# vghuy17ck1/svt-av1-psyex

Measured on AMD Instinct MI355X. Metric: ME+RD-cost Mpixels/s (2160p10 preset-6), higher is better.
Workload: dtype u8 SAD / i32 transforms; 1 GPU; 3840x2160 10-bit synthetic pan sequence, preset 6 (M6) search controls at qp 35; step = 16 pictures (4 current pictures x ref distance 1,2,4,8; R=2): open-loop ME of all 2040 b64 + full-pel pred + RD chain (64x64,32x32,16x16 DCT_DCT, 10-bit, b quantizer; qcoeff + recon + scalars written); 3 picture sets alternate from step to step

## Files before the change

svt-av1-psyex_amd/csrc/me_kernel.hip:

```cpp
#include <hip/hip_runtime.h>
#include <stdint.h>
#include <string.h>
#include "me_kernel.h"
#include "wave_ops.h"

#ifdef SVT_HIP_ME_PROFILE
struct Prof { uint32_t *acc; unsigned long long last; int step; };
#define SVT_HIP_ME_PROFILE_LDS (48 * 4)
#define PROF_DECL Prof prof_; prof_.acc = reinterpret_cast<uint32_t *>(g_lds + lay.total); if (threadIdx.x < 48) prof_.acc[threadIdx.x] = 0; prof_.last = __builtin_readcyclecounter(); prof_.step = 0; Prof *prof = &prof_
#define PROF_STEP(s) (prof->step = (s))
#define PROFS(i) PROF((i) + prof->step)
#define PROF(i) do { const unsigned long long t_ = __builtin_readcyclecounter(); if (threadIdx.x == 0) atomicAdd(&prof->acc[i], (uint32_t)(t_ - prof->last)); prof->last = t_; } while (0)
#define PROF_FLUSH(ptr) do { __builtin_amdgcn_fence(__ATOMIC_RELEASE, "wavefront"); if (threadIdx.x < 48) atomicAdd((unsigned long long *)(ptr) + threadIdx.x, (unsigned long long)prof->acc[threadIdx.x]); } while (0)
#define PROF_PARAM , Prof *prof
#define PROF_ARG , prof
#else
#define PROF_DECL do { } while (0)
#define PROF(i) do { } while (0)
#define PROFS(i) do { } while (0)
#define PROF_STEP(s) do { } while (0)
#define PROF_FLUSH(ptr) do { } while (0)
#define SVT_HIP_ME_PROFILE_LDS 0
#define PROF_PARAM
#define PROF_ARG
// ... 757 lines not shown
    best        = k < best ? k : best;
}

__device__ __attribute__((noinline)) void stage_clamped(uint8_t *win, const uint8_t *pix0, uint32_t stride, int min_x, int max_x, int min_y, int max_y, int wx0, int wy0,
                                                        int pitch, int rows) {
    for (int i = threadIdx.x; i < pitch * rows; i += kThreads) {
        const int row = i / pitch, cb = i - row * pitch;
        const int x = imin(imax(wx0 + cb, min_x), max_x), y = imin(imax(wy0 + row, min_y), max_y);
        win[row * pitch + cb] = pix0[x + (long long)y * stride];
    }
}

constexpr int kMeInFlight = 4;
constexpr int kMeOrdBits = 12;
__device__ __forceinline__ void run_me_searches(Shared &sh, CParams &p, const MeReq *list, int count, uint32_t *bsad, uint32_t *bmv, int r0n PROF_PARAM) {
    const int lane = threadIdx.x;
    const int sub  = (p.cfg.me_search_method == 0);
    const int nrow = sub ? 4 : 8, rstep = sub ? 2 : 1;
    const int g = lane >> 4, pu = lane & 15;
    const int bx = (pu & 1) | ((pu >> 1) & 2), by = ((pu >> 1) & 1) | ((pu >> 2) & 2);
    const uint8_t *srow = &LDS(sh.src64)[bx * 16];
    for (int mi = 0; mi < count; mi++) {
        MeReq m;
        {
            const MeReq &mm = list[mi];
            m.pix0 = uni_ptr(mm.pix0); m.stride = uni(mm.stride);
            m.ox = (int16_t)uni((uint32_t)mm.ox); m.oy = (int16_t)uni((uint32_t)mm.oy); m.sa_w = (int16_t)uni((uint32_t)mm.sa_w); m.sa_h = (int16_t)uni((uint32_t)mm.sa_h);
            m.li = (uint8_t)uni(mm.li); m.ri = (uint8_t)uni(mm.ri); m.probe = 0; m.pad = 0;
            m.min_x = (int16_t)uni((uint32_t)mm.min_x); m.max_x = (int16_t)uni((uint32_t)mm.max_x); m.min_y = (int16_t)uni((uint32_t)mm.min_y); m.max_y = (int16_t)uni((uint32_t)mm.max_y);
        }
        u64 b8[4] = {~0ull, ~0ull, ~0ull, ~0ull}, b16 = ~0ull, b32 = ~0ull, b64 = ~0ull;
        const int W = m.sa_w, H = m.sa_h;
        int       tw = W, th = H;
        auto me_pitch = [](int shift, int ww) { return ((shift + ww - 1 + 64 + 15) & ~15) + 16; };
        auto wbytes = [&](int ww, int hh) { return (uint32_t)me_pitch(0, ww) * (uint32_t)(hh - 1 + 64); };
        while (th > 1 && (wbytes(tw, th) > (uint32_t)kWinBytes || tw * th > (1 << kMeOrdBits))) th = (th + 1) >> 1;
        while (tw > 8 && (wbytes(tw, th) > (uint32_t)kWinBytes || tw * th > (1 << kMeOrdBits))) tw = ((tw >> 1) + 7) & ~7;
        for (int y0 = 0; y0 < H; y0 += th)
            for (int x0 = 0; x0 < W; x0 += tw) {
                const int w = imin(tw, W - x0), h = imin(th, H - y0);
                const uint8_t *gwin  = m.pix0 + (m.ox + x0) + (long long)(m.oy + y0) * m.stride;
                const int pitch = me_pitch(0, w);
                const int rows        = h - 1 + 64;
                const int vec_per_row = pitch >> 4;
                const float vpr_rcp   = rcp_of((uint32_t)vec_per_row);
                wave_sync();
                const int wx0 = m.ox + x0, wy0 = m.oy + y0;
                if (m.ox + x0 >= m.min_x && m.ox + x0 + w - 1 + 63 <= m.max_x && wy0 >= m.min_y && wy0 + rows - 1 <= m.max_y) {
                    const int nvec = vec_per_row * rows;
                    for (int b0 = 0; b0 < nvec; b0 += kMeInFlight * kThreads) {
                        const int base = b0 + lane;
                        int  k[kMeInFlight];
                        V4   v[kMeInFlight];
#pragma unroll
                        for (int j = 0; j < kMeInFlight; j++) {
                            if (b0 + j * kThreads < nvec) {
                                k[j] = imin(base + j * kThreads, nvec - 1);
                                const int row = (int)div_by_rcp((uint32_t)k[j], vpr_rcp), c = k[j] - row * vec_per_row;
                                const V4U q4 = *reinterpret_cast<GV4U *>(reinterpret_cast<uintptr_t>(gwin + (long long)row * m.stride + c * 16));
                                v[j] = V4{q4.x, q4.y, q4.z, q4.w};
                            }
                        }
#pragma unroll
                        for (int j = 0; j < kMeInFlight; j++)
                            if (b0 + j * kThreads < nvec) *reinterpret_cast<V4 *>(&LDS(sh.win)[k[j] * 16]) = v[j];
                    }
                } else {
                    stage_clamped(LDS(sh.win), m.pix0, m.stride, m.min_x, m.max_x, m.min_y, m.max_y, wx0, wy0, pitch, rows);
                }
                wave_sync();
                PROF(46);
                const int ng = (w + 3) >> 2;
                uint32_t k8[4] = {~0u, ~0u, ~0u, ~0u}, k16 = ~0u, k32 = ~0u, k64 = ~0u;
                const int kshift = kMeOrdBits + sub;
                for (int y = 0; y < h; y += 4) {
                    const bool live = y + g < h;
                    const int  yy   = live ? y + g : h - 1;
                    const uint8_t *wrow = &LDS(sh.win)[(yy + by * 16) * pitch + bx * 16];
                    const uint32_t ord0 = (uint32_t)(yy * w);
                    for (int gq = 0; gq < ng; gq++) {
                        const uint8_t *wp = wrow + 4 * gq;
                        u64 acc[4] = {0, 0, 0, 0};
#pragma unroll
                        for (int half = 0; half < 2; half++)
#pragma unroll
                            for (int k = 0; k < 8; k++) {
                                if (k < nrow) {
                                    const int r = 8 * half + k * rstep;
                                    const uint32_t *wr = reinterpret_cast<const uint32_t *>(wp + r * pitch);
                                    const uint32_t d0 = wr[0], d1 = wr[1], d2 = wr[2], d3 = wr[3], d4 = wr[4];
                                    const uint4 sv = *reinterpret_cast<const uint4 *>(srow + ((by * 16 + r) >> sh.cshift) * kSrc64Pitch);
                                    acc[2 * half] = __builtin_amdgcn_qsad_pk_u16_u8(((u64)d1 << 32) | d0, sv.x, acc[2 * half]);
                                    acc[2 * half] = __builtin_amdgcn_qsad_pk_u16_u8(((u64)d2 << 32) | d1, sv.y, acc[2 * half]);
                                    acc[2 * half + 1] = __builtin_amdgcn_qsad_pk_u16_u8(((u64)d3 << 32) | d2, sv.z, acc[2 * half + 1]);
                                    acc[2 * half + 1] = __builtin_amdgcn_qsad_pk_u16_u8(((u64)d4 << 32) | d3, sv.w, acc[2 * half + 1]);
                                }
                            }
#pragma unroll
                        for (int i = 0; i < 4; i++) {
                            const int x = 4 * gq + i;
                            uint32_t v8[4];
#pragma unroll
                            for (int j = 0; j < 4; j++) v8[j] = (uint32_t)((acc[j] >> (16 * i)) & 0xFFFF);
                            const uint32_t v16 = (v8[0] + v8[1]) + (v8[2] + v8[3]);
                            const uint32_t v32 = quad_sum(v16);
                            const uint32_t v64 = row16_sum_of_quads(v32);
                            if (x < w && live) {
                                const uint32_t ord = ord0 + (uint32_t)x;
#pragma unroll
                                for (int j = 0; j < 4; j++) k8[j] = umin32(k8[j], (v8[j] << kshift) | ord);
                                k16 = umin32(k16, (v16 << kshift) | ord);
                                k32 = umin32(k32, (v32 << kshift) | ord);
                                k64 = umin32(k64, (v64 << kshift) | ord);
                            }
                        }
                    }
                }
                PROF(47);
                const float w_rcp = rcp_of((uint32_t)w);
                auto fold = [&](u64 &best, uint32_t k) {
                    k = umin32(k, (uint32_t)__shfl_xor((int)k, 16, 64));
                    k = umin32(k, (uint32_t)__shfl_xor((int)k, 32, 64));
                    if (k != ~0u) {
                        const uint32_t ordl = k & ((1u << kMeOrdBits) - 1u), ty = div_by_rcp(ordl, w_rcp), tx = ordl - ty * (uint32_t)w;
                        upd(best, k >> kMeOrdBits, (uint32_t)((y0 + (int)ty) * W + (x0 + (int)tx)));
                    }
                };
#pragma unroll
                for (int j = 0; j < 4; j++) fold(b8[j], k8[j]);
                fold(b16, k16); fold(b32, k32); fold(b64, k64);
            }
        uint32_t *rs_ = bsad + ((m.li ? r0n : 0) + m.ri) * 85, *rm_ = bmv + ((m.li ? r0n : 0) + m.ri) * 85;
        auto merge = [&](int n, u64 k) {
            const uint32_t sad = (uint32_t)(k >> 32);
            if (k != ~0ull && sad < rs_[n]) {
                const uint32_t ord = (uint32_t)k;
                const int      yy = (int)(ord / (uint32_t)W), xx = (int)(ord - (uint32_t)yy * (uint32_t)W);
                rs_[n] = sad;
                rm_[n] = ((uint32_t)(m.oy + yy) << 16) | (uint16_t)(m.ox + xx);
            }
        };
        if (g == 0) {
#pragma unroll
            for (int j = 0; j < 4; j++) merge(21 + 4 * pu + j, b8[j]);
            merge(5 + pu, b16);
            if ((pu & 3) == 0) merge(1 + (pu >> 2), b32);
            if (pu == 0) merge(0, b64);
        }
        wave_sync();
    }
}


__device__ __forceinline__ bool searched(CParams &p, int li) { return p.desc.temporal_layer_index > 0 || li == 0; }

__device__ void set_hme_all(St &st, CParams &p, int lvl, int li, int ri, int x, int y, uint32_t sad) {
    for (int h = 0; h < p.cfg.num_hme_sa_h; h++)
        for (int w = 0; w < p.cfg.num_hme_sa_w; w++) {
            st.hx[lvl][li][ri][w][h] = (int16_t)x;
            st.hy[lvl][li][ri][w][h] = (int16_t)y;
            st.hs[lvl][li][ri][w][h] = sad;
        }
}

template <class P> __host__ __device__ __forceinline__ void hme_l0_area(P &p, int li, int ri, uint32_t dist, int mvx, int mvy, int &sa_w, int &sa_h) {
    auto &c = p.cfg;
    struct { SvtHipSearchAreaMinMax hme_l0_sa; } st;
    st.hme_l0_sa.sa_min.width = (uint16_t)c.hme_l0_sa.sa_min.width; st.hme_l0_sa.sa_min.height = (uint16_t)c.hme_l0_sa.sa_min.height;
    st.hme_l0_sa.sa_max.width = (uint16_t)c.hme_l0_sa.sa_max.width; st.hme_l0_sa.sa_max.height = (uint16_t)c.hme_l0_sa.sa_max.height;
    if (c.enable_me_sr_adjustment && c.distance_based_hme_resizing) {
        int is_hor = 1, is_ver = 1, is_still = 0;
        if (c.reduce_hme_l0_sr_th_min && c.reduce_hme_l0_sr_th_max && (li || ri)) {
            is_ver   = iabs(mvx) < c.reduce_hme_l0_sr_th_min && iabs(mvy) > c.reduce_hme_l0_sr_th_max;
            is_hor   = iabs(mvx) > c.reduce_hme_l0_sr_th_max && iabs(mvy) < c.reduce_hme_l0_sr_th_min;
            is_still = iabs(mvx) < c.reduce_hme_l0_sr_th_min * 3 && iabs(mvy) < c.reduce_hme_l0_sr_th_min * 3;
        }
        int xo = is_hor ? 1 : 2, yo = is_ver ? 1 : 2;
        if (c.enable_me_sr_adjustment == 2 && is_still) xo = yo = 4;
        st.hme_l0_sa.sa_min.width  = (uint16_t)(st.hme_l0_sa.sa_min.width / (xo + ri));
        st.hme_l0_sa.sa_min.height = (uint16_t)(st.hme_l0_sa.sa_min.height / (yo + ri));
        st.hme_l0_sa.sa_max.width  = (uint16_t)(st.hme_l0_sa.sa_max.width / (xo + ri));
        st.hme_l0_sa.sa_max.height = (uint16_t)(st.hme_l0_sa.sa_max.height / (yo + ri));
    }
    const int f = (int)scaled_distance(dist);
    int       w = (int16_t)(st.hme_l0_sa.sa_min.width / c.num_hme_sa_w);
    w           = (int16_t)imin(((w * f) + 15) & ~15, ((st.hme_l0_sa.sa_max.width / c.num_hme_sa_w) + 15) & ~15);
    int h       = (int16_t)(st.hme_l0_sa.sa_min.height / c.num_hme_sa_h);
    h           = (int16_t)imin(h * f, st.hme_l0_sa.sa_max.height / c.num_hme_sa_h);
    sa_w        = w;
    sa_h        = h;
}
__device__ void hme_l0_search_area(const St &cst, CParams &p, int li, int ri, uint32_t dist, int &sa_w, int &sa_h) {
    hme_l0_area(p, li, ri, dist, cst.hx[0][0][0][0][0], cst.hy[0][0][0][0][0], sa_w, sa_h);
}

template <class P> __host__ __device__ __forceinline__ void prehme_size(P &p, int li, int ri, int sri, int &sa_w, int &sa_h) {
    auto &c = p.cfg;
    const uint32_t f = scaled_distance(ref_distance(p, li, ri));
    sa_w = (int16_t)(uint16_t)imin((int)(c.prehme_sa_cfg[sri].sa_min.width * f), c.prehme_sa_cfg[sri].sa_max.width);
    sa_h = (int16_t)(uint16_t)imin((int)(c.prehme_sa_cfg[sri].sa_min.height * f), c.prehme_sa_cfg[sri].sa_max.height);
}
__device__ __forceinline__ SearchGeo prehme_geometry(CParams &p, int li, int ri, int sri, uint32_t org_x, uint32_t org_y) {
    int sa_w, sa_h;
    prehme_size(p, li, ri, sri, sa_w, sa_h);
    CPlane &rp = p.ref[li][ri].lvl[0];
    const int ox16 = (int16_t)org_x >> 2, oy16 = (int16_t)org_y >> 2;
    int ox = -(int16_t)(sa_w >> 1), oy = -(int16_t)(sa_h >> 1);
    clip_axis(ox16, ox, sa_w, rp.org_x - 1, rp.width);
    clip_axis(oy16, oy, sa_h, rp.org_y - 1, rp.height);
    SearchGeo g = {ox, oy, sa_w, sa_h};
    return g;
}

__device__ __forceinline__ SearchGeo hme_level_geometry(CParams &p, int level, CPlane &rp, int org_x, int org_y, int sa_w, int sa_h, int cx, int cy, int sr_w, int sr_h) {
    sa_w = (int16_t)((sa_w + 7) & ~7);
    int pad_w, pad_h, ox, oy;
    if (level == 2) { pad_w = pad_h = 63; } else { pad_w = rp.org_x - 1; pad_h = rp.org_y - 1; }
    if (level == 0) {
        ox = -(int16_t)((sa_w * p.cfg.num_hme_sa_w) >> 1) + (int16_t)(sa_w * sr_w);
        oy = -(int16_t)((sa_h * p.cfg.num_hme_sa_h) >> 1) + (int16_t)(sa_h * sr_h);
    } else {
        ox = -(sa_w >> 1) + cx;
        oy = -(sa_h >> 1) + cy;
    }
    clip_axis(org_x, ox, sa_w, pad_w, rp.width);
    sa_w = (sa_w < 8) ? sa_w : (sa_w & ~7);
    clip_axis(org_y, oy, sa_h, pad_h, rp.height);
    SearchGeo g = {ox, oy, sa_w, sa_h};
    return g;
}

struct HmeGeom { int16_t ox, oy; };

__device__ HmeGeom push_hme_level(St &st, CParams &p, int level, CPlane &rp, int org_x, int org_y, int bw, int bh,
                                  int sa_w, int sa_h, int cx, int cy, int sr_w, int sr_h, int slot = -1) {
    const SearchGeo sg = hme_level_geometry(p, level, rp, org_x, org_y, sa_w, sa_h, cx, cy, sr_w, sr_h);
    push_hme_req(st, p, level, rp, org_x, org_y, bw, bh, sg.ox, sg.oy, sg.sa_w, sg.sa_h, 0, slot);
    HmeGeom g = {(int16_t)sg.ox, (int16_t)sg.oy};
    return g;
}

__device__ __forceinline__ void key_to_result(u64 key, int full, uint32_t &sad, int &x, int &y) {
    sad = (uint32_t)(key >> 32);
    if ((uint32_t)key == 0xffffffffu) { x = 0; y = 0; }
    else { y = (int)((key >> 16) & 0xFFFF); x = (int)(key & 0xFFFF); }
    if (!full) sad *= 2;
}

__device__ __forceinline__ void push_zz_req(St &st, CPlane &rp, int dx, int dy, int slot = -1) {
    push_req(st, plane_at(rp, (int)st.org_x + dx, (int)st.org_y + dy), rp.stride, 1, 1, (int)st.b64_w, (int)st.b64_h >> 1, 2, 2, 0, slot);
}

}


#ifndef SVT_ME_CTRL_PRIO
#define SVT_ME_CTRL_PRIO 2
#endif
#define CTRL_PRIO(x) __builtin_amdgcn_s_setprio(x)

constexpr size_t kPersistBytes = (offsetof(St, req) + 15) & ~(size_t)15;
template <int MODE>
__device__ __forceinline__ void me_b64_body(const MeBatchHeader *__restrict__ ghdr, const MeKernelParams *__restrict__ gparams, const uint32_t launch_flags) {
    St     &st = *reinterpret_cast<St *>(g_lds);
    typedef const SVT_CONST_AS MeBatchHeader CHeader;
    CHeader  &hdr = *(CHeader *)ghdr;
    const int tid = threadIdx.x;
    const int       cshift = (int)hdr.cshift;
    const bool      has_dense = hdr.dense != nullptr;
    const LdsLayout lay    = lds_layout((int)hdr.n_slot, cshift, has_dense ? 1 : 0, MODE);
    uint32_t *const bsad = reinterpret_cast<uint32_t *>(g_lds + lay.bsad);
    uint32_t *const bmv  = reinterpret_cast<uint32_t *>(g_lds + lay.bmv);
    const MeDenseSlot *const dense_lds = has_dense ? reinterpret_cast<const MeDenseSlot *>(g_lds + lay.dense) : nullptr;
    uint32_t n_hit = 0, n_miss = 0;
    Shared sh = {st, lay.src64, lay.src32, lay.src16, lay.win, cshift};

    uint32_t xcc = 0;
    asm volatile("s_getreg_b32 %0, hwreg(HW_REG_XCC_ID)" : "=s"(xcc));
    xcc &= 7;
    int queue_probe = 0;
    constexpr int kList = 0;
    const bool list_mode = (launch_flags & 1u) != 0;
    const uint32_t n_total = hdr.job_base[hdr.n_pictures];
    uint32_t share_next = 0, share_end = 0, share_step = 1;
    if (MODE != kMeFull && !list_mode) {
        if (gridDim.x >= SVT_HIP_ME_QUEUES) {
            const uint32_t q = blockIdx.x % SVT_HIP_ME_QUEUES;
            share_step = (gridDim.x - q + SVT_HIP_ME_QUEUES - 1) / SVT_HIP_ME_QUEUES;
            share_next = hdr.queue_begin[q] + blockIdx.x / SVT_HIP_ME_QUEUES;
            share_end  = hdr.queue_begin[q + 1];
        } else {
            share_step = gridDim.x; share_next = blockIdx.x; share_end = n_total;
        }
    }
    auto fetch_job = [&]() {
        int job = -1;
        if (list_mode) {
            const uint32_t n = __hip_atomic_load(&hdr.queue_head[SVT_HIP_ME_LIST_COUNT(kList)], __ATOMIC_RELAXED, __HIP_MEMORY_SCOPE_AGENT);
            if (__hip_atomic_load(&hdr.queue_head[SVT_HIP_ME_LIST_CURSOR(kList)], __ATOMIC_RELAXED, __HIP_MEMORY_SCOPE_AGENT) >= n) return job;
            const uint32_t k = atomicAdd(&hdr.queue_head[SVT_HIP_ME_LIST_CURSOR(kList)], 1u);
            if (k < n) job = (int)hdr.lists[kList][k];
            return job;
        }
        if (MODE != kMeFull) {
            if (share_next < share_end) { job = (int)share_next; share_next += share_step; }
            return job;
// ... 478 lines not shown
            const bool mine = tid < 8 && li < nl && ri < d.num_of_ref_pic_to_search[li] && !(dep && ((li == 0 && ri == 0) != (gi == 0))) && st.do_ref[li][ri];
            MeReq m = {};
            if (mine) {
                CPlane &rp = p.ref[li][ri].lvl[2];
                int16_t  cx = st.me_cx[li][ri], cy = st.me_cy[li][ri];
                const uint32_t dist = mctf ? (uint16_t)ref_distance(p, li, ri) : (uint16_t)scaled_distance(ref_distance(p, li, ri));
                int16_t sa_w = (int16_t)imin((int)(c.me_sa.sa_min.width * dist), c.me_sa.sa_max.width);
                int16_t sa_h = (int16_t)imin((int)(c.me_sa.sa_min.height * dist), c.me_sa.sa_max.height);
                if (c.mv_sa_adj_enabled && (!c.mv_sa_adj_nearest_ref_only || ri == 0)) {
                    if (iabs(st.hme_sc_x[li][ri]) > c.mv_sa_adj_mv_size_th) sa_w = (int16_t)(sa_w * c.mv_sa_adj_sa_multiplier);
                    if (iabs(st.hme_sc_y[li][ri]) > c.mv_sa_adj_mv_size_th) sa_h = (int16_t)(sa_h * c.mv_sa_adj_sa_multiplier);
                }
                { const uint32_t q = (uint32_t)(int)sa_w / st.sr_divisor[li][ri]; sa_w = (int16_t)(((q > 1u ? q : 1u) + 7) & ~7u); }
                { const uint32_t q = (uint32_t)(int)sa_h / st.sr_divisor[li][ri]; sa_h = (int16_t)(q > 3u ? q : 3u); }
                const int16_t h0 = sa_h, w0 = sa_w;
                u64 best_hme_sad = ~0ull;
                if (c.me_early_exit_th) {
                    if (st.zz_sad[li][ri] < c.me_early_exit_th / 6) sa_w = sa_h = 1;
                } else {
                    int accurate = 1;
                    const int k2 = st.c00_req[li][ri];
                    if (k2) {
                        const uint32_t zero = (uint32_t)(st.req_key[k2 - 2] >> 32) << 1;
                        const uint32_t hme  = (uint32_t)(st.req_key[k2 - 1] >> 32) << 1;
                        if (zero <= hme) cx = cy = 0;
                        best_hme_sad = hme;
                        if (cx == 0 && cy == 0) accurate = 0;
                    }
                    if (c.enable_me_sr_adjustment == 2) {
                        if ((accurate && best_hme_sad < 24 * 24) || (d.is_ref && st.hme_sad64[li][ri] < 24 * 24)) sa_h = (int16_t)(sa_h / 2);
                        if ((li || ri) && BEST_SAD(0, 0)[0] < 5000 && sa_h == h0 && sa_w == w0) { sa_h = (int16_t)(sa_h >> 1); sa_w = (int16_t)(sa_w >> 1); }
                    }
                }
                m.pix0 = plane_at(rp, (int)st.org_x, (int)st.org_y); m.stride = rp.stride;
                m.min_x = (int16_t)(-rp.org_x - (int)st.org_x); m.max_x = (int16_t)(rp.width + rp.org_x - 1 - (int)st.org_x);
                m.min_y = (int16_t)(-rp.org_y - (int)st.org_y); m.max_y = (int16_t)(rp.height + rp.org_y - 1 - (int)st.org_y);
                m.li = (uint8_t)li; m.ri = (uint8_t)ri; m.pad = 0;
                m.sa_w = sa_w; m.sa_h = sa_h;
                m.ox = cx; m.oy = cy;
                m.probe = (c.me_8x8_var_enabled && sa_w * sa_h > 24) ? 1 : 0;
            }
            const bool probe = mine && m.probe;
            const u64  mask = __ballot(mine), pmask = __ballot(probe), below = (1ull << tid) - 1ull;
            if (mine) st.me[__popcll(mask & below)] = m;
            if (probe) { MeReq pr = m; pr.sa_w = pr.sa_h = 1; st.me_probe[__popcll(pmask & below)] = pr; }
            if (tid == 0) { st.nme = __popcll(mask); st.nprobe = __popcll(pmask); }
        };
        auto main_pre = [&]() {
            if (tid < 64) {
                const int pic_w = (int16_t)d.aligned_width, pic_h = (int16_t)d.aligned_height;
                for (int i = 0; i < st.nme; i++) {
                    const MeReq m = st.me[i];
                    int16_t sa_w = m.sa_w, sa_h = m.sa_h;
                    const int cx = m.ox, cy = m.oy;
                    if (m.probe) {
                        const uint32_t mean = BEST_SAD(m.li, m.ri)[0] / 64;
                        const int32_t  dd   = (int32_t)BEST_SAD(m.li, m.ri)[21 + tid] - (int32_t)mean;
                        const uint32_t var  = wave_sum((uint32_t)(dd * dd)) / 64;
                        if (var > c.me_sr_mult2_th) { sa_w = (int16_t)((imax(1, sa_w * 3 / 2) + 7) & ~7); sa_h = (int16_t)imax(1, sa_h * 3 / 2); }
                        if (var < c.me_sr_div4_th) { sa_w = (int16_t)((imax(1, sa_w >> 2) + 7) & ~7); sa_h = (int16_t)imax(3, imax(1, sa_h >> 2)); }
                        else if (var < c.me_sr_div2_th) { sa_w = (int16_t)((imin(sa_w, sa_w >> 1) + 7) & ~7); sa_h = (int16_t)imax(3, imin(sa_h, sa_h >> 1)); }
                    }
                    int ox = (int16_t)(cx - (sa_w >> 1)), oy = (int16_t)(cy - (sa_h >> 1)), w = sa_w, h = sa_h;
                    clip_axis((int16_t)st.org_x, ox, w, 63, pic_w);
                    w = (w < 8) ? w : (w & ~7);
                    clip_axis((int16_t)st.org_y, oy, h, 63, pic_h);
                    if (tid == 0) { MeReq &o = st.me[i]; o.ox = (int16_t)ox; o.oy = (int16_t)oy; o.sa_w = (int16_t)w; o.sa_h = (int16_t)h; }
                }
            }
        };

        enum { kZz, kPrehme, kL0, kL1, kL2, kC00, kProbe, kMain, kEnd };
#ifdef SVT_ME_ABLATE
        if (SVT_ME_ABLATE == 1) continue;
#endif
        const int n_prehme = c.prehme_l1_early_exit ? nl : 1, n_l0 = l0_dep ? 2 : 1, n_group = me_dep ? 2 : 1;
        if constexpr (MODE == kMeMid1 || MODE == kMeMid2) {
            const bool hme_on = c.enable_hme_flag;
            bool defer = false;
            uint32_t flags = 0;
            if constexpr (MODE == kMeMid1) {
                auto pending = [&]() { return __any(tid < st.nreq && !st.req[tid].done); };
                if (c.me_early_exit_th || c.me_safe_limit_zz_th) { zz_pre(); wave_sync(); zz_post(); wave_sync(); }
                if (c.prehme_enable) {
                    for (int b2 = 0; b2 < n_prehme; b2++) {
                        prehme_pre(b2); wave_sync();
                        if (pending()) { defer = true; break; }
                        prehme_post(b2);
                        if (b2 + 1 < n_prehme) wave_sync();
                    }
                    if (!defer) { prehme_final(); wave_sync(); }
                }
                if (!defer && hme_on && c.enable_hme_level0_flag)
                    for (int b2 = 0; b2 < n_l0; b2++) {
                        l0_pre(b2); wave_sync();
                        if (pending()) { defer = true; break; }
                        l0_post(b2); wave_sync();
                    }
                if (!defer) {
                    if (hme_on && c.enable_hme_level1_flag) lvl_pre(1);
                    else if (tid == 0) st.nreq = 0;
                    wave_sync();
                }
            } else {
                flags = __hip_atomic_load(jflag, __ATOMIC_RELAXED, __HIP_MEMORY_SCOPE_AGENT);
                if (hme_on && c.enable_hme_level1_flag) { lvl_post(1); wave_sync(); }
                if (hme_on && c.enable_hme_level2_flag) lvl_pre(2);
                else if (tid == 0) st.nreq = 0;
                wave_sync();
            }
            if (!defer && st.nreq && !small_direct_ok(st)) defer = true;
            if (defer) {
                if (tid == 0) {
                    *jflag = SVT_HIP_ME_JOB_DEFERRED;
                    hdr.lists[0][atomicAdd(&hdr.queue_head[SVT_HIP_ME_LIST_COUNT(0)], 1u)] = (uint32_t)gjob;
                }
            } else {
                export_state(gjob);
                export_reqs(gjob);
                if (tid == 0) *jflag = flags;
            }
            wave_sync();
            continue;
        }
        if constexpr (MODE == kMeTail) {
            if (c.enable_hme_flag && c.enable_hme_level2_flag) { lvl_post(2); wave_sync(); }
        }
        int step = MODE == kMeTail ? kC00 : kZz, bi = 0;
        PROF(2);
        while (step != kEnd) {
            bool run = true;
            CTRL_PRIO(SVT_ME_CTRL_PRIO);
            switch (step) {
            case kZz: run = c.me_early_exit_th || c.me_safe_limit_zz_th; if (run) zz_pre(); break;
            case kPrehme: run = c.prehme_enable; if (run) prehme_pre(bi); break;
            case kL0: run = c.enable_hme_flag && c.enable_hme_level0_flag; if (run) l0_pre(bi); break;
            case kL1: run = c.enable_hme_flag && c.enable_hme_level1_flag; if (run) lvl_pre(1); break;
            case kL2: run = c.enable_hme_flag && c.enable_hme_level2_flag; if (run) lvl_pre(2); break;
            case kC00: if (bi == 0) centre(); c00_pre(bi); break;
            case kProbe: probe_pre(bi); break;
            default: main_pre(); break;
            }
#ifdef SVT_ME_ABLATE
            if (SVT_ME_ABLATE == 2 && step == kC00) break;
            if (SVT_ME_ABLATE >= 10 && step == SVT_ME_ABLATE - 10) break;
            if (SVT_ME_ABLATE == 4 && run && step < kProbe) { step = step == kPrehme ? kL0 : step + 1; bi = 0; continue; }
            if (SVT_ME_ABLATE == 5 && run && step < kProbe) st.nreq = 0;
#endif
            if (run) {
                CTRL_PRIO(0);
                wave_sync();
                PROF(step == kMain ? 20 : 6 + step);
                if (step == kC00 && bi == 0 && st.tf_exit) { step = kEnd; continue; }
                if (step < kProbe) {
                    PROF_STEP(step);
                    if (st.nreq) {
                        if (!run_small_searches_direct(sh PROF_ARG)) run_searches(sh PROF_ARG);
                    }
                } else {
                    const bool   probe = step == kProbe;
                    const MeReq *list  = probe ? st.me_probe : st.me;
                    const int    count = probe ? st.nprobe : st.nme;
                    run_me_searches(sh, p, list, count, bsad, bmv, r0n PROF_ARG);
                }
                PROF(step == kProbe ? 3 : step == kMain ? 4 : 19);
            }
            CTRL_PRIO(SVT_ME_CTRL_PRIO);
            switch (step) {
            case kZz: if (run) zz_post(); step = kPrehme; break;
            case kPrehme:
                if (run) prehme_post(bi);
                if (run && bi + 1 < n_prehme) { bi++; break; }
                if (run) prehme_final();
                step = kL0; bi = 0;
                break;
            case kL0:
                if (run) l0_post(bi);
                if (run && bi + 1 < n_l0) { bi++; break; }
                step = kL1; bi = 0;
                break;
            case kL1: if (run) lvl_post(1); step = kL2; break;
            case kL2: if (run) lvl_post(2); step = kC00; break;
            case kC00: step = kProbe; break;
            case kProbe: step = kMain; break;
            default:
                if (bi + 1 < n_group) { bi++; step = kC00; } else step = kEnd;
                break;
            }
            CTRL_PRIO(0);
            wave_sync();
            PROF(5);
        }


#ifdef SVT_ME_ABLATE
        if (SVT_ME_ABLATE == 2 || SVT_ME_ABLATE == 3 || SVT_ME_ABLATE >= 10) continue;
#endif
        if (c.enable_hme_flag && c.enable_me_hme_ref_pruning && !mctf) {
            for (int r = 0; r < 8; r++) {
                const int li = r >> 2, ri = r & 3;
                if (li >= nl || ri >= d.num_of_ref_pic_to_search[li]) continue;
                const u64 t = st.do_ref[li][ri] ? (u64)wave_sum(BEST_SAD(li, ri)[21 + (tid & 63)]) : (u64)SVT_HIP_MAX_SAD_VALUE * 64;
                if ((tid & 63) == 0) st.hme_sad64[li][ri] = t;
            }
            wave_sync();
            {
                const uint16_t th = c.prune_ref_if_me_sad_dev_bigger_than_th;
                if (th != 0xFFFF) {
                    const int  li = (tid >> 2) & 1, ri = tid & 3;
                    const bool slot = tid < 8;
                    const u64  hs = slot ? st.hme_sad64[li][ri] : ~0ull;
                    const u64  best = (u64)wave_min_dpp((uint32_t)(hs < 0xFFFFFFFFull ? hs : 0xFFFFFFFFull));
                    if (slot && ri >= 1 && (hs - best) * 100 > (u64)th * best) st.do_ref[li][ri] = 0;
                }
            }
            wave_sync();
        }

        PROF(13);
        {
          if (!mctf) {
            const uint32_t n_pu = p.n_pu;
            uint8_t  *o_total = p.res.total_me_candidate_index + (size_t)b * n_pu;
            uint32_t *o_mv    = p.res.me_mv_array + (size_t)b * n_pu * d.max_refs;
            uint8_t  *o_cand  = p.res.me_candidate_array + (size_t)b * n_pu * d.max_cand;
            const int r0 = d.num_of_ref_pic_to_search[0], r1 = d.num_of_ref_pic_to_search[1];
            auto use_pu = [&](int nn) { return d.enable_me_16x16 ? (d.enable_me_8x8 || nn < 21) : nn < 5; };
            auto pack   = [](unsigned dir, unsigned i0, unsigned i1, unsigned l0, unsigned l1) {
                return (uint8_t)((dir & 3) | ((i0 & 3) << 2) | ((i1 & 3) << 4) | ((l0 & 1) << 6) | ((l1 & 1) << 7));
            };
            uint32_t *l_mv    = reinterpret_cast<uint32_t *>(LDS(sh.win));
            uint8_t  *l_cand  = LDS(sh.win) + 4 * n_pu * d.max_refs;
            uint8_t  *l_total = l_cand + n_pu * d.max_cand;
            const int stage_dwords = (int)(4 * n_pu * d.max_refs + n_pu * d.max_cand + n_pu + 3) >> 2;
            static_assert(kWinBytes >= 85 * (4 * SVT_HIP_MAX_LISTS * SVT_HIP_MAX_REFS + 32 + 1), "the result rows of one block fit the arena");
            for (int i = tid; i < stage_dwords; i += kThreads) reinterpret_cast<uint32_t *>(LDS(sh.win))[i] = 0;
            wave_sync();
            for (int n = tid; n < d.max_number_of_pus_per_sb; n += kThreads) {
                const int use = use_pu(n);
                const int row = (n > 4) ? c_z_to_raster[n] : n;
                uint8_t first = 0;
                auto put_cand = [&](int idx, uint8_t v) { l_cand[row * d.max_cand + idx] = v; if (idx == 0) first = v; };
                uint32_t  nls = nl;
                if (r0 == 1 && r1 == 0) {
                    const int pu   = c_z_to_raster[n];
                    st.me_dist[pu] = BEST_SAD(0, 0)[n];
                    if (use) l_total[pu] = 1;
                    if (st.do_ref[0][0] && use) { put_cand(0, pack(0, 0, 0, 0, 0)); l_mv[pu * d.max_refs] = BEST_MV(0, 0)[n]; }
                } else if (r0 == 1 && r1 == 1) {
                    const int     pu = c_z_to_raster[n];
                    const uint8_t d0 = st.do_ref[0][0], d1 = (nls == 1) ? 0 : st.do_ref[1][0];
                    if (nls < 2 || !st.do_ref[1][0]) nls = 1;
                    const uint32_t prune_th = (d0 && d1) ? (uint32_t)c.prune_me_candidates_th : 0;
                    uint8_t  blk[2] = {d0, d1};
                    uint8_t  off = 0;
                    const uint32_t s0 = BEST_SAD(0, 0)[n], s1 = BEST_SAD(1, 0)[n];
                    const uint32_t best = (d0 && d1) ? (s0 < s1 ? s0 : s1) : (d0 ? s0 : s1);
                    st.me_dist[pu] = best;
                    if (use) l_total[pu] = 1;
                    int min_list = -1;
                    if (c.use_best_unipred_cand_only && blk[0] && blk[1]) min_list = s0 < s1 ? 0 : 1;
                    for (uint32_t li = 0; li < nls && (use || off == 0); li++) {
                        if (!blk[li]) continue;
                        if (prune_th > 0) {
                            const uint32_t dev = (BEST_SAD(li, 0)[n] - best) * 100;
                            if (dev > best * prune_th) { blk[li] = 0; continue; }
                        }
                        if (min_list != -1 && min_list != (int)li) {
                            if (use) l_mv[pu * d.max_refs + (li ? d.max_l0 : 0)] = BEST_MV(li, 0)[n];
                            continue;
                        }
                        if (use) {
                            put_cand(off, pack(li, 0, 0, li == 0 ? li : 24, li == 1 ? li : 24));
                            l_mv[pu * d.max_refs + (li ? d.max_l0 : 0)] = BEST_MV(li, 0)[n];
                        }
                        off++;
                    }
                    if (blk[0] && blk[1] && use) { put_cand(off, pack(2, 0, 0, 0, 1)); l_total[pu] = (uint8_t)(off + 1); }
                } else {
                    const int pu = (n > 4) ? c_z_to_raster[n] : n;
                    uint8_t   off = 0;
                    uint8_t   blk[2][4] = {{0, 0, 0, 0}, {0, 0, 0, 0}};
                    const uint32_t prune_th = (uint32_t)c.prune_me_candidates_th;
                    uint32_t       best     = ~0u;
                    for (uint32_t li = 0; li < nls; li++)
                        for (int ri = 0; ri < d.num_of_ref_pic_to_search[li]; ri++) {
                            blk[li][ri] = st.do_ref[li][ri];
                            if (blk[li][ri]) best = BEST_SAD(li, ri)[n] < best ? BEST_SAD(li, ri)[n] : best;
                        }
                    st.me_dist[pu] = best;
                    for (uint32_t li = 0; li < nls && (use || off == 0); li++)
                        for (int ri = 0; ri < d.num_of_ref_pic_to_search[li] && (use || off == 0); ri++) {
                            if (!blk[li][ri]) continue;
                            if (prune_th > 0) {
                                const uint32_t dev = (BEST_SAD(li, ri)[n] - best) * 100;
                                if (dev > best * prune_th) { blk[li][ri] = 0; continue; }
                            }
                            if (use) {
                                put_cand(off, pack(li, ri, ri, li == 0 ? li : 24, li == 1 ? li : 24));
                                l_mv[pu * d.max_refs + (li ? d.max_l0 : 0) + ri] = BEST_MV(li, ri)[n];
                            }
                            off++;
                        }
                    if (nls == 2 && use) {
                        for (int a = 0; a < r0; a++)
                            for (int bb = 0; bb < r1; bb++) {
                                if (d.only_l_bwd && (a > 0 || bb > 0)) continue;
// ... 314 lines not shown
```

Baseline: 40150 Mpixels/s.

## Add specialized batched SAD paths for C00 and probe steps in ME tail mode

```diff
diff --git a/svt-av1-psyex_amd/csrc/me_kernel.hip b/svt-av1-psyex_amd/csrc/me_kernel.hip
--- a/svt-av1-psyex_amd/csrc/me_kernel.hip
+++ b/svt-av1-psyex_amd/csrc/me_kernel.hip
@@ -933,6 +933,120 @@
 }
 
 
+constexpr int kC00Round = 8;
+__device__ __forceinline__ void c00_sads(Shared &sh) {
+    St &st = sh.st;
+    const int lane = threadIdx.x;
+    const int nreq = (int)uni((uint32_t)st.nreq), bw = (int)uni(st.b64_w), bh = (int)uni(st.b64_h);
+    for (int q0 = 0; q0 < nreq; q0 += kC00Round) {
+        V4 w[kC00Round][2];
+#pragma unroll
+        for (int j = 0; j < kC00Round; j++)
+            if (q0 + j < nreq) {
+                const uint8_t *win = uni_ptr(st.req[q0 + j].win);
+                const uint32_t stride = uni(st.req[q0 + j].stride);
+#pragma unroll
+                for (int h = 0; h < 2; h++) {
+                    const int i = lane + 64 * h, y = (i >> 2) * 2, x = (i & 3) * 16;
+                    w[j][h] = V4{0, 0, 0, 0};
+                    if (y < bh && x < bw) w[j][h] = __builtin_bit_cast(V4, *reinterpret_cast<GV4U *>(reinterpret_cast<uintptr_t>(win + (long long)y * stride + x)));
+                }
+            }
+#pragma unroll
+        for (int j = 0; j < kC00Round; j++)
+            if (q0 + j < nreq) {
+                uint32_t a = 0;
+#pragma unroll
+                for (int h = 0; h < 2; h++) {
+                    const int i = lane + 64 * h, y = (i >> 2) * 2, x = (i & 3) * 16;
+                    if (y < bh && x < bw) {
+                        const V4 v = *reinterpret_cast<const V4 *>(&LDS(sh.src64)[(y >> sh.cshift) * kSrc64Pitch + x]);
+                        a = __builtin_amdgcn_sad_u8(v.x, w[j][h].x, a);
+                        a = __builtin_amdgcn_sad_u8(v.y, w[j][h].y, a);
+                        if (x + 8 < bw) { a = __builtin_amdgcn_sad_u8(v.z, w[j][h].z, a); a = __builtin_amdgcn_sad_u8(v.w, w[j][h].w, a); }
+                    }
+                }
+                const uint32_t t = wave_sum_dpp(a);
+                if (lane == 0) st.req_key[q0 + j] = (u64)t << 32;
+            }
+    }
+    wave_sync();
+}
+
+typedef uint32_t V2 __attribute__((ext_vector_type(2)));
+typedef uint32_t V2U __attribute__((ext_vector_type(2), aligned(1)));
+typedef const __attribute__((address_space(1))) V2U GV2U;
+
+constexpr int kProbeRound = 4;
+__device__ __forceinline__ void probe_sads(Shared &sh, CParams &p, uint32_t *bsad, uint32_t *bmv, int r0n PROF_PARAM) {
+    St &st = sh.st;
+    const int lane = threadIdx.x;
+    const int sub  = (p.cfg.me_search_method == 0);
+    const int nrow = sub ? 4 : 8, rstep = sub ? 2 : 1;
+    const int px = 8 * ((lane & 1) | ((lane >> 1) & 2) | ((lane >> 2) & 4)), py = 8 * (((lane >> 1) & 1) | ((lane >> 2) & 2) | ((lane >> 3) & 4));
+    const int count = (int)uni((uint32_t)st.nprobe);
+    for (int m0 = 0; m0 < count; m0 += kProbeRound) {
+        V2 w[kProbeRound][8];
+#pragma unroll
+        for (int j = 0; j < kProbeRound; j++)
+            if (m0 + j < count) {
+                const MeReq &mm = st.me_probe[m0 + j];
+                const uint8_t *pix0 = uni_ptr(mm.pix0);
+                const uint32_t stride = uni(mm.stride);
+                const int ox = (int16_t)uni((uint32_t)mm.ox), oy = (int16_t)uni((uint32_t)mm.oy);
+                const int min_x = (int16_t)uni((uint32_t)mm.min_x), max_x = (int16_t)uni((uint32_t)mm.max_x);
+                const int min_y = (int16_t)uni((uint32_t)mm.min_y), max_y = (int16_t)uni((uint32_t)mm.max_y);
+                if (ox >= min_x && ox + 63 <= max_x && oy >= min_y && oy + 63 <= max_y) {
+                    const uint8_t *g = pix0 + (ox + px) + (long long)(oy + py) * stride;
+#pragma unroll
+                    for (int k = 0; k < 8; k++)
+                        if (k < nrow) w[j][k] = __builtin_bit_cast(V2, *reinterpret_cast<GV2U *>(reinterpret_cast<uintptr_t>(g + (long long)(k * rstep) * stride)));
+                }
+            }
+        PROF(17);
+#pragma unroll
+        for (int j = 0; j < kProbeRound; j++)
+            if (m0 + j < count) {
+                const MeReq &mm = st.me_probe[m0 + j];
+                const int ox = (int16_t)uni((uint32_t)mm.ox), oy = (int16_t)uni((uint32_t)mm.oy);
+                const int row = (uni(mm.li) ? r0n : 0) + (int)uni(mm.ri);
+                const int min_x = (int16_t)uni((uint32_t)mm.min_x), max_x = (int16_t)uni((uint32_t)mm.max_x);
+                const int min_y = (int16_t)uni((uint32_t)mm.min_y), max_y = (int16_t)uni((uint32_t)mm.max_y);
+                uint32_t a = 0;
+                if (ox >= min_x && ox + 63 <= max_x && oy >= min_y && oy + 63 <= max_y) {
+#pragma unroll
+                    for (int k = 0; k < 8; k++)
+                        if (k < nrow) {
+                            const V2 s = *reinterpret_cast<const V2 *>(&LDS(sh.src64)[((py + k * rstep) >> sh.cshift) * kSrc64Pitch + px]);
+                            a = __builtin_amdgcn_sad_u8(s.x, w[j][k].x, a);
+                            a = __builtin_amdgcn_sad_u8(s.y, w[j][k].y, a);
+                        }
+                } else {
+                    const uint8_t *pix0 = uni_ptr(mm.pix0);
+                    const uint32_t stride = uni(mm.stride);
+#pragma nounroll
+                    for (int i = 0; i < nrow * 8; i++) {
+                        const int k = i >> 3, b = i & 7;
+                        const int x = imin(imax(ox + px + b, min_x), max_x), y = imin(imax(oy + py + k * rstep, min_y), max_y);
+                        a += (uint32_t)iabs((int)LDS(sh.src64)[((py + k * rstep) >> sh.cshift) * kSrc64Pitch + px + b] - (int)*reinterpret_cast<const __attribute__((address_space(1))) uint8_t *>(reinterpret_cast<uintptr_t>(pix0 + x + (long long)y * stride)));
+                    }
+                }
+                const uint32_t v8 = a << sub, v16 = quad_sum(v8), v32 = row16_sum_of_quads(v16), v64 = wave_sum_dpp(v8);
+                uint32_t *rs_ = bsad + row * 85, *rm_ = bmv + row * 85;
+                const uint32_t mv = ((uint32_t)oy << 16) | (uint16_t)ox;
+                auto merge = [&](int n, uint32_t sad) {
+                    if (sad < rs_[n]) { rs_[n] = sad; rm_[n] = mv; }
+                };
+                merge(21 + lane, v8);
+                if ((lane & 3) == 0) merge(5 + (lane >> 2), v16);
+                if ((lane & 15) == 0) merge(1 + (lane >> 4), v32);
+                if (lane == 0) merge(0, v64);
+            }
+    }
+    wave_sync();
+}
+
+
 __device__ __forceinline__ bool searched(CParams &p, int li) { return p.desc.temporal_layer_index > 0 || li == 0; }
 
 __device__ void set_hme_all(St &st, CParams &p, int lvl, int li, int ri, int x, int y, uint32_t sad) {
@@ -1717,7 +1831,16 @@
                 wave_sync();
                 PROF(step == kMain ? 20 : 6 + step);
                 if (step == kC00 && bi == 0 && st.tf_exit) { step = kEnd; continue; }
-                if (step < kProbe) {
+                if constexpr (MODE == kMeTail) {
+                    if (step == kC00) {
+                        c00_sads(sh);
+                        PROF(18);
+                    } else if (step == kProbe) {
+                        probe_sads(sh, p, bsad, bmv, r0n PROF_ARG);
+                    } else {
+                        run_me_searches(sh, p, st.me, st.nme, bsad, bmv, r0n PROF_ARG);
+                    }
+                } else if (step < kProbe) {
                     PROF_STEP(step);
                     if (st.nreq) {
                         if (!run_small_searches_direct(sh PROF_ARG)) run_searches(sh PROF_ARG);
```

Measured after the change: 40780 Mpixels/s (median of 6 runs). 1.02x the previous value.
